# leonsick/s2d

Measured on AMD Instinct MI355X. Metric: clip-frames/sec fwd+loss, R50 M2F-Video T=8 720p Q=100, higher is better.
Workload: dtype f32 (f16x3 MFMA for dense contractions); 1 GPU; KDVideoMaskFormer fwd+loss (student+teacher fwd, GT+KD VideoSetCriterion), c4: 2 clips/GPU x T=8 x 720x1280, Q=100, P=160000, N=10 sparse GT instances/clip, encoder dropout 0.3; clips_per_gpu=2, frames_per_clip=8, parallelism=dp1 (clips sharded, no collective), streams=2

## Files before the change

### include/s2d_hip.h

```cpp
#ifndef S2D_HIP_H
#define S2D_HIP_H
#include <stdint.h>

#ifndef HIP_INCLUDE_HIP_HIP_RUNTIME_API_H
typedef struct ihipStream_t *hipStream_t;
#endif

#ifdef __cplusplus
extern "C" {
#endif

#define S2D_OK 0
#define S2D_ERR_ARG (-1)
#define S2D_ERR_LAUNCH (-2)

int s2d_abi_version(void);

int s2d_set_dense_mode(int mode);


int s2d_gemm_nt_f32(const float *A, const float *B, float *C, int M, int N, int K, long lda, long ldb, long ldc,
                    int batch, long strideA, long strideB, long strideC, const float *scale, const float *bias,
                    const float *res, long ldr, long strideR, int res_rows, int res_cols, int relu, const void *B_split,
                    hipStream_t stream);
// ... 259 lines not shown

int s2d_relu_gate_add_f32(const float *a, const float *g, const float *y, long n, float *out, hipStream_t stream);


int s2d_optim_grad_norm_f32(const void *const *ptrs, const long *numel, const int *chunk_tensor, const long *chunk_off,
                            int nchunks, int chunk, float inv_scale, float max_norm, double *partial, float *normbuf,
                            hipStream_t stream);

int s2d_optim_adamw_ema_f32(const void *const *ptrs, const long *numel, const double *hyper, const int *chunk_tensor,
                            const long *chunk_off, int nchunks, int chunk, double lr_factor, double beta1, double beta2,
                            double eps, double bias_correction1, double bias_correction2_sqrt, float inv_scale, double ema_m,
                            const float *normbuf, hipStream_t stream);

int s2d_point_loss_backward_f32(const float *mask_logits, const uint8_t *tgt, const int *tgt_count, const int *nonempty,
                                const int *idx_q, const int *idx_t, const int *n_match, const float *coords_over,
                                const float *coords_rand, uint64_t seed, int NL, int B, int Q, int ldq, int T, int hm, int wm,
                                int H, int W, int Nmax, int num_points, float oversample_ratio, float importance_ratio,
                                int drop_empty, float world_size, void *workspace, float w_mask, float w_dice, float *grad_rows,
                                unsigned int *bit_scratch, hipStream_t stream);

int s2d_point_loss_rng_points(uint64_t seed, int hm, int wm, int row0, int nrows, int n_over, float *uv, int *bounds, int *scratch_list,
                              hipStream_t stream);

int s2d_class_loss_backward_f32(const float *class_logits, const int *idx_q, const int *n_match, int B, int Q, int maxm,
                                float eos_coef, float w_ce, float *d_class_logits, hipStream_t stream);

int s2d_class_loss_backward_c_f32(const float *class_logits, int C1, const int *idx_q, const int *n_match, int B, int Q, int maxm,
                                  float eos_coef, float w_ce, float *d_class_logits, hipStream_t stream);


int s2d_tracks_to_masks_u8(const float *tracks, int T, int Np, int H, int W, uint8_t *masks, hipStream_t stream);

int s2d_point_id_counts(const uint8_t *point_masks, const int64_t *idmap, int T, int H, int W, int Hi, int Wi, int max_id,
                        int *counts, int *total, hipStream_t stream);

int s2d_track_point_id_counts(const float *tracks, int T, int P, int H, int W, const int64_t *idmap, int Hi, int Wi, int max_id,
                              int *counts, int *total, hipStream_t stream);

int s2d_idmap_select_masks_u8(const int64_t *idmap, int T, int H, int W, const int *frames, const int *objs, int K, uint8_t *out,
                              hipStream_t stream);

int s2d_idmap_presence_u8(const int64_t *idmap, int T, int Hi, int Wi, int max_id, uint8_t *presence, hipStream_t stream);

long s2d_color_ids_workspace_words(int T);
int s2d_color_masks_to_ids(const uint8_t *rgb, int T, int H, int W, unsigned int *workspace, int *n_ids, int64_t *ids,
                           int *overflow, hipStream_t stream);
// ... 64 lines not shown
```

### s2d_amd/csrc/loss.hip

```cpp
#include "common.h"
#include "class_select.h"

namespace {

__device__ __forceinline__ uint64_t mix64(uint64_t z)
{
    z += 0x9E3779B97F4A7C15ull;
    z = (z ^ (z >> 30)) * 0xBF58476D1CE4E5B9ull;
    z = (z ^ (z >> 27)) * 0x94D049BB133111EBull;
    return z ^ (z >> 31);
}
__device__ __forceinline__ uint32_t hash32(uint32_t x)
{
    x ^= x >> 16; x *= 0x7feb352du; x ^= x >> 15; x *= 0x846ca68bu; x ^= x >> 16;
    return x;
}
__device__ __forceinline__ uint32_t rand_key(uint64_t seed, uint64_t stream)
{
    return (uint32_t)mix64(seed ^ mix64(stream * 0xD1342543DE82EF95ull));
}
__device__ __forceinline__ uint32_t rand_u_bits(uint32_t key, uint32_t i) { return hash32(key + i); }
__device__ __forceinline__ uint32_t rand_v_bits(uint32_t a)
{
    uint32_t b = a * 0x9E3779B1u;
// ... 178 lines not shown
    const int *nonempty;
    const int *idx_q, *idx_t;
    const int *n_match;
    const float *coords_over;
    const float *coords_rand;
    uint64_t seed;
    int NL, B, Q, ldq, T, hm, wm, H, W, Nmax, maxm, n_over, n_unc, n_rand, drop;
    float world_size;
    int *active, *rank;
    int *list;
    int *lcount;
    float *mq;
    unsigned int *hist;
    unsigned int *prefix;
    int *krem;
    unsigned int *tie;
    float *part;
    int chunks;
    float *xbuf;
    unsigned int *tpack;
    int bits_global;
    int xcap;
    int *pbound;
};

__device__ __forceinline__ uint64_t key_row(const LossParams &p, long rowid)
{
    if (p.NL == 0) return (uint64_t)rowid;
    const long per = (long)p.maxm * p.T;
    const long lb = rowid / per;
    return (uint64_t)(lb * ((long)p.Q * p.T) + (rowid - lb * per));
}

constexpr int PB_STRIDE = 9;
struct VRange {
    float v0, dv;
};

__global__ void row_prep_kernel(LossParams p)
{
    const int layer = blockIdx.x;
    const int rows_l = p.B * p.maxm * p.T;
    __shared__ int base;
    if (threadIdx.x == 0) base = 0;
    __syncthreads();
    for (int r0 = 0; r0 < rows_l; r0 += blockDim.x) {
        const int r = r0 + threadIdx.x;
        int act = 0;
        if (r < rows_l) {
            const int t = r % p.T, s = (r / p.T) % p.maxm, b = r / (p.T * p.maxm);
            const int prob = layer * p.B + b;
            if (s < p.n_match[prob]) {
                const int n = p.idx_t[(long)prob * p.maxm + s];
                act = p.drop ? p.nonempty[((long)b * p.Nmax + n) * p.T + t] : 1;
            }
        }
        __shared__ int wsum[4];
        const unsigned long long m = __ballot(act);
        const int lane = threadIdx.x & 63, wv = threadIdx.x >> 6;
        const int inw = __popcll(m & ((1ull << lane) - 1ull));
        if (lane == 0) wsum[wv] = __popcll(m);
        __syncthreads();
        int off = base;
        for (int w = 0; w < wv; ++w) off += wsum[w];
        if (r < rows_l) {
            const long rowid = (long)layer * rows_l + r;
            p.active[rowid] = act;
// ... 271 lines not shown
{
    extern __shared__ __attribute__((aligned(16))) float smem[];
    __shared__ int hq_idx[LTHREADS / 64][128];
    __shared__ float hq_y[LTHREADS / 64][128];
    constexpr int nb = LEVEL == 0 ? 2048 : 1024;
    const PartGeom g = part_geom(p.hm, p.wm);
    unsigned int *h = reinterpret_cast<unsigned int *>(smem);
    float *sm = smem + 2048;
    PartIter it(p, g.nparts, LEVEL == 0 ? 0 : p.xcap);
    long rowid; int part, li;
    while (it.next(p, rowid, part, li)) {
        __syncthreads();
        for (int i = threadIdx.x; i < nb; i += LTHREADS) h[i] = 0u;
        const int r0 = part * g.rows_per_part;
        const int nr = min(g.rows_per_part + 1, p.hm - r0);
        const float *cr = coord_rows(p, rowid, true);
        const bool padded = cr == nullptr;
        const int wp = p.wm + 2 * PADC;
        if (padded) stage_part_padded(p.mq + rowid * p.hm * p.wm, p.wm, r0, nr, sm);
        else stage_part(p.mq + rowid * p.hm * p.wm, p.wm, r0, nr, sm);
        __syncthreads();
        const unsigned int pre = LEVEL > 0 ? p.prefix[rowid] : 0u;
        const uint32_t key0 = rand_key(p.seed, key_row(p, rowid) * 2);
        const int ylo = part == 0 ? -1 : r0, yhi = r0 + g.rows_per_part;
        auto tally = [&](int i, float xv) {
            const unsigned int key = __float_as_uint(fabsf(xv));
            if (LEVEL == 0 && li < p.xcap && !(S2D_LOSS_DBG & 4)) p.xbuf[(long)li * (p.n_over + p.n_rand) + i] = xv;
            if ((S2D_LOSS_DBG & 1) && LEVEL == 0) { if (key == 0x12345u) h[0] = 1u; return; }
            if (LEVEL == 0) atomicAdd(&h[key >> 20], 1u);
            else if (LEVEL == 1) { if ((key >> 20) == (pre >> 20)) atomicAdd(&h[(key >> 10) & 1023u], 1u); }
            else { if ((key >> 10) == (pre >> 10)) atomicAdd(&h[key & 1023u], 1u); }
        };
        if (!cr) {
            const int *pb = p.pbound + rowid * PB_STRIDE;
            const int lo = pb[part], hi = pb[part + 1];
            const VRange vr = part_vrange(part, g.nparts, g.rows_per_part, p.hm);
            const int y0max = min(yhi, p.hm) - 1;
#pragma unroll 2
            for (int i = lo + (int)threadIdx.x; i < hi; i += LTHREADS) {
                const uint32_t ra_ = rand_u_bits(key0, (uint32_t)i);
                const float u = (float)(ra_ >> 8) * (1.0f / 16777216.0f);
                const float v = fmaf((float)(rand_v_bits(ra_) >> 8) * (1.0f / 16777216.0f), vr.dv, vr.v0);
                const float y = ((2.f * v - 1.f + 1.f) * p.hm - 1.f) * 0.5f;
                const float x = ((2.f * u - 1.f + 1.f) * p.wm - 1.f) * 0.5f;
                const int y0 = min(max((int)floorf(y), ylo), y0max);
                if (S2D_LOSS_DBG & 2) tally(i, x * y + (float)y0); else
                tally(i, sample_part_padded(sm, wp, r0, x, y, (int)floorf(x), y0));
            }
        } else {
            const int lane = threadIdx.x & 63, wv = threadIdx.x >> 6;
            int *qi = hq_idx[wv];
            float *qy = hq_y[wv];
// ... 34 lines not shown
            const uint32_t key1 = rand_key(p.seed, key_row(p, rowid) * 2 + 1);
            for (int i = threadIdx.x; i < p.n_rand; i += LTHREADS) {
                float u, v;
                if (cr2) { u = cr2[2 * i]; v = cr2[2 * i + 1]; }
                else {
                    const uint32_t ra_ = rand_u_bits(key1, (uint32_t)i);
                    u = (float)(ra_ >> 8) * (1.0f / 16777216.0f);
                    v = (float)(rand_v_bits(ra_) >> 8) * (1.0f / 16777216.0f);
                }
                const float y = ((2.f * v - 1.f + 1.f) * p.hm - 1.f) * 0.5f;
                const float x = ((2.f * u - 1.f + 1.f) * p.wm - 1.f) * 0.5f;
                const int y0 = (int)floorf(y);
                if (y0 >= ylo && y0 < yhi)
                    p.xbuf[(long)li * (p.n_over + p.n_rand) + p.n_over + i] =
                        padded ? sample_part_padded(sm, wp, r0, x, y, (int)floorf(x), y0) : sample_part(sm, p.hm, p.wm, r0, nr, x, y, (int)floorf(x), y0);
            }
        }
        __syncthreads();
        for (int i = threadIdx.x; i < nb; i += LTHREADS)
            if (h[i]) atomicAdd(&p.hist[rowid * 2048 + i], h[i]);
    }
}

template <int LEVEL>
__global__ __launch_bounds__(256) void hist_stream_kernel(LossParams p)
{
    __shared__ unsigned int h[1024];
    constexpr int SCH = 8;
    const int nrows = min(p.lcount[p.NL], p.xcap);
    for (int w = blockIdx.x; w < nrows * SCH; w += gridDim.x) {
        const int li = w / SCH, chunk = w % SCH;
        const long rowid = p.list[li];
        __syncthreads();
        for (int i = threadIdx.x; i < 1024; i += 256) h[i] = 0u;
        __syncthreads();
        const unsigned int pre = p.prefix[rowid];
        const float *xb = p.xbuf + (long)li * (p.n_over + p.n_rand);
        const int per = ((p.n_over + SCH - 1) / SCH + 3) & ~3;
        const int i0 = chunk * per, i1 = min(p.n_over, i0 + per);
        for (int i = i0 + threadIdx.x * 4; i < i1; i += 256 * 4) {
            const f32x4 v = *reinterpret_cast<const f32x4 *>(xb + i);
#pragma unroll
            for (int j = 0; j < 4; ++j) {
                if (i + j >= i1) break;
                const unsigned int key = __float_as_uint(fabsf(v[j]));
                if (LEVEL == 1) { if ((key >> 20) == (pre >> 20)) atomicAdd(&h[(key >> 10) & 1023u], 1u); }
                else { if ((key >> 10) == (pre >> 10)) atomicAdd(&h[key & 1023u], 1u); }
            }
        }
        __syncthreads();
        for (int i = threadIdx.x; i < 1024; i += 256)
            if (h[i]) atomicAdd(&p.hist[rowid * 2048 + i], h[i]);
    }
}

template <bool COH = false>
__device__ __forceinline__ float sample_bits(const unsigned int *bits, int H, int W, float u, float v)
{
    const float gx = 2.f * u - 1.f, gy = 2.f * v - 1.f;
    const float x = ((gx + 1.f) * W - 1.f) * 0.5f, y = ((gy + 1.f) * H - 1.f) * 0.5f;
    const int x0 = (int)floorf(x), y0 = (int)floorf(y), x1 = x0 + 1, y1 = y0 + 1;
    const float fx = x - x0, fy = y - y0;
    const float wxa = (x0 >= 0 && x0 < W) ? 1.f - fx : 0.f, wxb = (x1 >= 0 && x1 < W) ? fx : 0.f;
    const float wya = (y0 >= 0 && y0 < H) ? 1.f - fy : 0.f, wyb = (y1 >= 0 && y1 < H) ? fy : 0.f;
    const int xa = min(max(x0, 0), W - 1), xb = min(max(x1, 0), W - 1);
    const int ya = min(max(y0, 0), H - 1) * W, yb = min(max(y1, 0), H - 1) * W;
    auto bit = [&](int idx) {
        const unsigned int w = COH ? __hip_atomic_load(bits + (idx >> 5), __ATOMIC_RELAXED, __HIP_MEMORY_SCOPE_AGENT) : bits[idx >> 5];
        return (float)((w >> (idx & 31)) & 1u);
    };
    float acc = bit(ya + xa) * (wxa * wya);
    acc += bit(ya + xb) * (wxb * wya);
    acc += bit(yb + xa) * (wxa * wyb);
    acc += bit(yb + xb) * (wxb * wyb);
    return acc;
}

template <int LEVEL>
__global__ __launch_bounds__(256) void select_kernel(LossParams p)
{
    __shared__ unsigned int csum[256];
    if ((int)blockIdx.x >= p.lcount[p.NL]) return;
    const long rowid = p.list[blockIdx.x];
    const int nb = LEVEL == 0 ? 2048 : 1024, per = nb / 256;
    const int k = LEVEL == 0 ? p.n_unc : p.krem[rowid];
    unsigned int *h = p.hist + rowid * 2048;
    unsigned int loc[8], s = 0;
    for (int j = 0; j < per; ++j) { loc[j] = h[threadIdx.x * per + j]; s += loc[j]; }
    csum[threadIdx.x] = s;
    __syncthreads();
    if (threadIdx.x == 0) {
        unsigned int run = 0;
        for (int i = 0; i < 256; ++i) { const unsigned int c = csum[i]; csum[i] = run; run += c; }
    }
    __syncthreads();
    unsigned int before = csum[threadIdx.x];
    if (k == 0 && LEVEL == 0 && threadIdx.x == 0) { p.prefix[rowid] = 0u; p.krem[rowid] = 0; }
    for (int j = 0; j < per; ++j) {
        if (before < (unsigned)k && before + loc[j] >= (unsigned)k) {
            const unsigned int bin = threadIdx.x * per + j;
            const unsigned int pre = LEVEL == 0 ? 0u : p.prefix[rowid];
            p.prefix[rowid] = LEVEL == 0 ? (bin << 20) : LEVEL == 1 ? (pre | (bin << 10)) : (pre | bin);
            p.krem[rowid] = k - (int)before;
        }
        before += loc[j];
    }
    __syncthreads();
    for (int j = 0; j < per; ++j) h[threadIdx.x * per + j] = 0u;
}

__device__ __forceinline__ void acc_point(float x, float t, float &bce, float &sgt, float &sg, float &ts)
{
    const float e = __expf(-fabsf(x));
    const float inv = __builtin_amdgcn_rcpf(1.f + e);
    const float s = x >= 0.f ? inv : e * inv;
    bce += fmaxf(x, 0.f) - x * t + __logf(1.f + e);
    sgt += s * t; sg += s; ts += t;
}

__global__ __launch_bounds__(LTHREADS) void accumulate_kernel(LossParams p)
{
    extern __shared__ __attribute__((aligned(16))) float smem[];
    __shared__ float red[LTHREADS / 64][4];
    const PartGeom g = part_geom(p.hm, p.wm);
    float *sm = smem;
    const int rows_l = p.B * p.maxm * p.T;
    PartIter it(p, g.nparts, p.xcap);
    long rowid; int part, li;
    while (it.next(p, rowid, part, li)) {
        __syncthreads();
        const int r0 = part * g.rows_per_part;
// ... 87 lines not shown
        out |= ((w4 & 0xFFu) ? 1u : 0u) << (4 * k);
        out |= ((w4 & 0xFF00u) ? 1u : 0u) << (4 * k + 1);
        out |= ((w4 & 0xFF0000u) ? 1u : 0u) << (4 * k + 2);
        out |= ((w4 & 0xFF000000u) ? 1u : 0u) << (4 * k + 3);
    }
    p.tpack[(long)plane * wpp + wd] = out;
}

struct LossBwdArgs {
    float *gplane;
    float w_mask, w_dice;
    unsigned int *bit_scratch;
};
template <bool BWD, bool GBITS = BWD>
__global__ __launch_bounds__(LTHREADS) void accumulate_stream_kernel(LossParams p, LossBwdArgs ba)
{
    extern __shared__ __attribute__((aligned(16))) unsigned int tbits[];
    __shared__ float red[LTHREADS / 64][4];
    constexpr int TIECAP = 512;
    __shared__ unsigned int tie_n, tie_base, wtie[LTHREADS / 64];
    __shared__ int tie_idx[TIECAP], tie_sorted[TIECAP];
    __shared__ int cq_idx[LTHREADS / 64][128];
    __shared__ float cq_val[LTHREADS / 64][128];
    const int rows_l = p.B * p.maxm * p.T;
    const int nrows = min(p.lcount[p.NL], p.xcap);
    const long HW = (long)p.H * p.W;
    __shared__ float s_v0[PB_STRIDE], s_dv[PB_STRIDE];
    __shared__ int s_pb[PB_STRIDE];
    const PartGeom sg_ = part_geom(p.hm, p.wm);
    if ((int)threadIdx.x < sg_.nparts) { const VRange vr = part_vrange(threadIdx.x, sg_.nparts, sg_.rows_per_part, p.hm); s_v0[threadIdx.x] = vr.v0; s_dv[threadIdx.x] = vr.dv; }
    static_assert(GBITS || !BWD, "the backward keeps its gradient tile in the dynamic LDS");
    const unsigned int *tb = tbits;
    int *gh = reinterpret_cast<int *>(tbits);
    const float n_pts = (float)(p.n_unc + p.n_rand);
    const bool injected = p.coords_over != nullptr || p.coords_rand != nullptr;
    const float FX_CAP = injected ? fmaxf(n_pts, 1.f) : fminf(fmaxf(n_pts, 1.f), fmaxf(1024.f, 256.f * n_pts / (float)(p.hm * p.wm)));
    __shared__ unsigned int tie_before;
    for (int li = blockIdx.x; li < nrows; li += gridDim.x) {
        const long rowid = p.list[li];
        const int layer = (int)(rowid / rows_l);
        const int r = (int)(rowid % rows_l);
        const int t = r % p.T, s = (r / p.T) % p.maxm, b = r / (p.T * p.maxm);
        const int prob = layer * p.B + b;
        const int n = p.idx_t[(long)prob * p.maxm + s];
        const unsigned int *pk = p.tpack + (((long)b * p.Nmax + n) * p.T + t) * (HW / 32);
        __syncthreads();
        if (threadIdx.x < PB_STRIDE) s_pb[threadIdx.x] = p.pbound[rowid * PB_STRIDE + threadIdx.x];
        if constexpr (GBITS) tb = pk;
        else {
#pragma unroll 4
            for (long w4 = threadIdx.x; w4 < HW / 128; w4 += LTHREADS) reinterpret_cast<uint4 *>(tbits)[w4] = reinterpret_cast<const uint4 *>(pk)[w4];
            for (long wd = (HW / 128) * 4 + threadIdx.x; wd < HW / 32; wd += LTHREADS) tbits[wd] = pk[wd];
        }
        if (threadIdx.x == 0) { tie_n = 0u; tie_base = 0u; }
        __syncthreads();
        const unsigned int thr = p.prefix[rowid];
        const unsigned int take = (unsigned int)p.krem[rowid];
        const float *xb = p.xbuf + (long)li * (p.n_over + p.n_rand);
        float bce = 0.f, sgt = 0.f, sg = 0.f, ts = 0.f;
        float g_bce = 0.f, g_dice = 0.f, dA = 0.f, dD = 1.f, fx_scale = 0.f, fx_inv = 0.f;
        float *gp = nullptr;
        if constexpr (BWD) {
            double num = 0.;
            for (int bb = 0; bb < p.B; ++bb) num += (double)min(p.tgt_count[bb], p.Nmax);
            num = fmax(num / (double)p.world_size, 1.0);
            float a = 0.f, bsum = 0.f, c = 0.f;
            for (int ch = 0; ch < p.chunks; ++ch) {
                const float *qd = p.part + (rowid * p.chunks + ch) * 4;
                a += qd[1]; bsum += qd[2]; c += qd[3];
            }
            dA = 2.f * a + 1.f; dD = bsum + c + 1.f;
            g_bce = ba.w_mask / ((float)num * (float)(p.n_unc + p.n_rand));
            g_dice = ba.w_dice / (float)num;
            gp = ba.gplane + rowid * (long)p.hm * p.wm;
            const float gmax = fabsf(g_bce) + fabsf(g_dice) * (2.f * dD + fabsf(dA)) / (4.f * dD * dD);
            fx_scale = gmax > 0.f ? exp2f(floorf(log2f(2147483648.f / (FX_CAP * gmax)))) : 0.f;
            fx_inv = fx_scale > 0.f ? 1.f / fx_scale : 0.f;
        }
        int ylo = 0, yhi = p.hm;
        int own_lo = -1, own_hi = p.hm;
// ... 74 lines not shown
                }
                point(xv, sample_bits(tb, p.H, p.W, u, v), u, v);
            };
            const int lane = threadIdx.x & 63, wv = threadIdx.x >> 6;
            int *qi = cq_idx[wv];
            float *qx = cq_val[wv];
            int qn = 0;
            auto push = [&](bool sel, int i, float xv) {
                const unsigned long long m = __ballot(sel);
                if (sel) {
                    const int pos = qn + (int)__popcll(m & ((1ull << lane) - 1ull));
                    qi[pos] = i; qx[pos] = xv;
                }
                qn += (int)__popcll(m);
                if (qn >= 64) {
                    heavy(qi[lane], qx[lane]);
                    const int rest = qn - 64;
                    int ti = 0; float tx = 0.f;
                    if (lane < rest) { ti = qi[64 + lane]; tx = qx[64 + lane]; }
                    if (lane < rest) { qi[lane] = ti; qx[lane] = tx; }
                    qn = rest;
                }
            };
            auto test = [&](int i, float xv, bool live) {
                const bool inr = live && i >= lo && i < hi;
                bool owned = inr;
                if (BWD && !walk_range && inr) {
                    float v;
                    if (cr) v = cr[2 * i + 1];
                    else if (over) { float u; over_point_rng(key0, i, s_pb, s_v0, s_dv, sg_.nparts, u, v); }
                    else v = (float)(rand_v_bits(rand_u_bits(key0, (uint32_t)i)) >> 8) * (1.0f / 16777216.0f);
                    const int y0 = y0_of(v);
                    owned = y0 >= own_lo && y0 < own_hi;
                }
                bool sel = owned;
                if (over) {
                    const unsigned int key = __float_as_uint(fabsf(xv));
                    sel = owned && key < thr;
                    if (inr && key == thr) {
                        const unsigned int slot = atomicAdd(&tie_n, 1u);
                        if (slot < TIECAP) tie_idx[slot] = i;
                    }
                }
                push(sel, i, xv);
            };
            const int cnt4 = ((reinterpret_cast<uintptr_t>(xs) & 15) == 0) ? cnt >> 2 : 0;
            const int b4 = min(lo >> 2, cnt4), e4 = min((hi + 3) >> 2, cnt4);
            const int it4 = (e4 - b4 + LTHREADS - 1) / LTHREADS;
            auto load4 = [&](int k) {
                const int i4 = b4 + k * LTHREADS + threadIdx.x;
                f32x4 x4 = {0.f, 0.f, 0.f, 0.f};
                if (i4 < e4) x4 = *reinterpret_cast<const f32x4 *>(xs + 4 * i4);
                return x4;
            };
            constexpr int DEPTH = 8;
            f32x4 ring[DEPTH];
#pragma unroll
            for (int d = 0; d < DEPTH; ++d) ring[d] = load4(d);
            for (int k0 = 0; k0 < it4; k0 += DEPTH) {
#pragma unroll
                for (int d = 0; d < DEPTH; ++d) {
                    const int k = k0 + d;
                    if (k >= it4) break;
                    const int i4 = b4 + k * LTHREADS + threadIdx.x;
                    const bool live = i4 < e4;
                    const f32x4 x4 = ring[d];
                    ring[d] = load4(k + DEPTH);
#pragma unroll
                    for (int j = 0; j < 4; ++j) test(4 * i4 + j, x4[j], live);
                }
            }
            const int tail0 = 4 * cnt4, itt = (cnt - tail0 + LTHREADS - 1) / LTHREADS;
            for (int k = 0; k < itt; ++k) {
                const int i = tail0 + k * LTHREADS + threadIdx.x;
                const bool live = i < cnt;
                test(i, live ? xs[i] : 0.f, live);
            }
            if (lane < qn) heavy(qi[lane], qx[lane]);
        }
        __syncthreads();
        const unsigned int nties = tie_n;
        const bool ranged_ties = BWD && ranged;
        const unsigned int before = ranged_ties ? tie_before : 0u;
        __syncthreads();
        if (ranged_ties && threadIdx.x == 0) tie_before = before + nties;
        if (nties > 0u && take > before) {
            const float *cr = coord_rows(p, rowid, true);
            const uint32_t key0 = rand_key(p.seed, key_row(p, rowid) * 2);
            auto tie_point = [&](int i) {
                float u, v;
                if (cr) { u = cr[2 * i]; v = cr[2 * i + 1]; }
                else over_point_rng(key0, i, s_pb, s_v0, s_dv, sg_.nparts, u, v);
                if (BWD && !ranged_ties) { const int y0 = y0_of(v); if (y0 < own_lo || y0 >= own_hi) return; }
                point(xb[i], sample_bits(tb, p.H, p.W, u, v), u, v);
            };
            if (nties <= (unsigned int)TIECAP) {
                for (unsigned int j = threadIdx.x; j < nties; j += LTHREADS) {
                    const int mine = tie_idx[j];
                    unsigned int rank = 0u;
// ... 28 lines not shown
            __syncthreads();
            const int nxt = part + 1 < nparts_b ? max((part + 1) * sg_.rows_per_part - 1, 0) : p.hm;
            for (int i = threadIdx.x; i < (min(nxt, yhi) - ylo) * p.wm; i += LTHREADS) gp[ylo * p.wm + i] = (float)gh[i] * fx_inv;
        }
        }
        if constexpr (!BWD) {
            bce = wave_sum(bce); sgt = wave_sum(sgt); sg = wave_sum(sg); ts = wave_sum(ts);
            const int lane = threadIdx.x & 63, wv = threadIdx.x >> 6;
            if (lane == 0) { red[wv][0] = bce; red[wv][1] = sgt; red[wv][2] = sg; red[wv][3] = ts; }
            __syncthreads();
            if (threadIdx.x < 4) {
                const int j = threadIdx.x;
                float tot = 0.f;
#pragma unroll
                for (int w = 0; w < LTHREADS / 64; ++w) tot += red[w][j];
                p.part[(rowid * p.chunks + 0) * 4 + j] = tot;
#pragma unroll 1
                for (int c = 1; c < p.chunks; ++c) p.part[(rowid * p.chunks + c) * 4 + j] = 0.f;
            }
        }
    }
}

__global__ void loss_finalize_kernel(LossParams p, float *__restrict__ losses)
{
    const int layer = blockIdx.x;
    if (threadIdx.x != 0) return;
    const int rows_l = p.B * p.maxm * p.T;
    double num = 0.;
    for (int b = 0; b < p.B; ++b) num += (double)min(p.tgt_count[b], p.Nmax);
    num = fmax(num / (double)p.world_size, 1.0);
    const double P = (double)(p.n_unc + p.n_rand);
    double lm = 0., ld = 0.;
    for (int r = 0; r < rows_l; ++r) {
        const long rowid = (long)layer * rows_l + r;
        if (!p.active[rowid]) continue;
        double bce = 0., sgt = 0., sg = 0., ts = 0.;
        for (int c = 0; c < p.chunks; ++c) {
            const float *q = p.part + (rowid * p.chunks + c) * 4;
            bce += q[0]; sgt += q[1]; sg += q[2]; ts += q[3];
        }
        lm += bce / P;
        ld += 1.0 - (2.0 * sgt + 1.0) / (sg + ts + 1.0);
    }
    losses[layer * 2 + 0] = (float)(lm / num);
    losses[layer * 2 + 1] = (float)(ld / num);
// ... 203 lines not shown

int s2d_target_nonempty(const uint8_t *tgt, const int *count, int B, int Nmax, int T, int H, int W, int *nonempty,
                        hipStream_t stream)
{
    if (B * Nmax * T == 0) return S2D_OK;
    if (((long)H * W) % 16) return S2D_ERR_ARG;
    if (s2d_zero_async(nonempty, sizeof(int) * (size_t)B * Nmax * T, stream) != S2D_OK) return S2D_ERR_LAUNCH;
    hipLaunchKernelGGL(nonempty_kernel, dim3(B * Nmax * T, NE_CHUNKS), dim3(256), 0, stream, tgt, count, Nmax, T, (long)H * W, nonempty);
    S2D_CHECK_LAUNCH();
    return S2D_OK;
}

static const int LOSS_CHUNKS = 8;

static const long XBUF_MAX_ROWS = 4096;

static void point_counts(int num_points, float oversample_ratio, float importance_ratio, int &n_over, int &n_unc, int &n_rand)
{
    n_over = (int)(num_points * oversample_ratio);
    n_unc = (int)(importance_ratio * num_points);
    n_rand = num_points - n_unc;
}

static inline bool plane_in_lds(long HW) { return HW / 8 <= 140 * 1024; }
constexpr int ACC_BLOCKS = 512;

long s2d_point_loss_workspace_bytes(int NL, int B, int Q, int Nmax, int T, int hm, int wm, int num_points,
                                    float oversample_ratio, float importance_ratio, int H, int W)
{
    const long maxm = Q < Nmax ? Q : Nmax;
    const long rows = (long)NL * B * maxm * T;
    int n_over, n_unc, n_rand;
    point_counts(num_points, oversample_ratio, importance_ratio, n_over, n_unc, n_rand);
    const long xrows = rows < XBUF_MAX_ROWS ? rows : XBUF_MAX_ROWS;
    const long HW = (long)H * W;
    return rows * (3 * 4 + (long)hm * wm * 4 + 2048 * 4 + 4 + 4 + 4 + LOSS_CHUNKS * 16 + PB_STRIDE * 4) + 4L * (NL + 1) + 1024 +
           xrows * (long)(n_over + n_rand + 8) * 4 + 256 + (long)B * Nmax * T * (HW / 32 + 1) * 4;
}

static int loss_setup(LossParams &p, long &rows, const float *mask_logits, const uint8_t *tgt, const int *tgt_count, const int *nonempty,
                      const int *idx_q, const int *idx_t, const int *n_match, const float *coords_over, const float *coords_rand,
                      uint64_t seed, int NL, int B, int Q, int ldq, int T, int hm, int wm, int H, int W, int Nmax, int num_points,
                      float oversample_ratio, float importance_ratio, int drop_empty, float world_size, void *workspace)
{
    if (Q > 128 || Nmax > 128 || ldq > 128 || ldq < Q || (ldq & 3)) return S2D_ERR_ARG;
    p.ml = mask_logits; p.tgt = tgt; p.tgt_count = tgt_count; p.nonempty = nonempty;
    p.idx_q = idx_q; p.idx_t = idx_t; p.n_match = n_match; p.coords_over = coords_over; p.coords_rand = coords_rand;
    p.seed = seed; p.NL = NL; p.B = B; p.Q = Q; p.ldq = ldq; p.T = T; p.hm = hm; p.wm = wm; p.H = H; p.W = W; p.Nmax = Nmax;
    p.maxm = Q < Nmax ? Q : Nmax;
    point_counts(num_points, oversample_ratio, importance_ratio, p.n_over, p.n_unc, p.n_rand);
    p.drop = drop_empty; p.world_size = world_size; p.chunks = LOSS_CHUNKS;
    rows = (long)NL * B * p.maxm * T;
    if (rows == 0) return S2D_OK;
    char *w = (char *)workspace;
    p.active = (int *)w; w += rows * 4;
    p.rank = (int *)w; w += rows * 4;
    p.prefix = (unsigned int *)w; w += rows * 4;
    p.krem = (int *)w; w += rows * 4;
    p.tie = (unsigned int *)w; w += rows * 4;
    p.list = (int *)w; w += rows * 4;
    p.lcount = (int *)w; w += 4L * (NL + 1);
    w = (char *)(((uintptr_t)w + 255) & ~(uintptr_t)255);
    p.hist = (unsigned int *)w; w += rows * 2048 * 4;
    p.part = (float *)w; w += rows * LOSS_CHUNKS * 16;
    p.pbound = (int *)w; w += rows * PB_STRIDE * 4;
    p.mq = (float *)w; w += rows * (long)hm * wm * 4;
    w = (char *)(((uintptr_t)w + 255) & ~(uintptr_t)255);
    p.xbuf = (float *)w;
    const bool can_stream = (p.n_over % 4 == 0) && (p.n_rand % 4 == 0) && ((long)H * W % 32 == 0);
    p.xcap = can_stream ? (int)(rows < XBUF_MAX_ROWS ? rows : XBUF_MAX_ROWS) : 0;
    {
        char *e = (char *)p.xbuf + (long)(rows < XBUF_MAX_ROWS ? rows : XBUF_MAX_ROWS) * (p.n_over + p.n_rand + 8) * 4;
        p.tpack = (unsigned int *)(((uintptr_t)e + 255) & ~(uintptr_t)255);
    }
    p.bits_global = can_stream && !plane_in_lds((long)H * W);
    const PartGeom pg = part_geom(hm, wm);
    if ((wm & 3) || pg.rows_per_part < 1 || pg.nparts > LOSS_CHUNKS) return S2D_ERR_ARG;
    p.chunks = pg.nparts;
    return S2D_OK;
}

static int loss_attrs()
{
    static S2dDevOnce attr_set;
    if (!attr_set.done()) {
        const int cap = PART_BYTES + 8192 + 4096;
        if (hipFuncSetAttribute(reinterpret_cast<const void *>(hist_kernel<0>), hipFuncAttributeMaxDynamicSharedMemorySize, cap) != hipSuccess ||
            hipFuncSetAttribute(reinterpret_cast<const void *>(hist_kernel<1>), hipFuncAttributeMaxDynamicSharedMemorySize, cap) != hipSuccess ||
            hipFuncSetAttribute(reinterpret_cast<const void *>(hist_kernel<2>), hipFuncAttributeMaxDynamicSharedMemorySize, cap) != hipSuccess ||
            hipFuncSetAttribute(reinterpret_cast<const void *>(accumulate_kernel), hipFuncAttributeMaxDynamicSharedMemorySize, cap) != hipSuccess ||
            hipFuncSetAttribute(reinterpret_cast<const void *>(accumulate_stream_kernel<false>), hipFuncAttributeMaxDynamicSharedMemorySize, 140 * 1024) != hipSuccess ||
            hipFuncSetAttribute(reinterpret_cast<const void *>(accumulate_stream_kernel<false, true>), hipFuncAttributeMaxDynamicSharedMemorySize, 140 * 1024) != hipSuccess ||
            hipFuncSetAttribute(reinterpret_cast<const void *>(accumulate_stream_kernel<true>), hipFuncAttributeMaxDynamicSharedMemorySize, 140 * 1024) != hipSuccess)
            return S2D_ERR_LAUNCH;
        attr_set.mark();
    }
    return S2D_OK;
}

int s2d_point_loss_f32(const float *mask_logits, const uint8_t *tgt, const int *tgt_count, const int *nonempty,
                       const int *idx_q, const int *idx_t, const int *n_match, const float *coords_over,
                       const float *coords_rand, uint64_t seed, int NL, int B, int Q, int ldq, int T, int hm, int wm, int H,
                       int W, int Nmax, int num_points, float oversample_ratio, float importance_ratio, int drop_empty,
                       float world_size, void *workspace, float *losses, hipStream_t stream)
{
    LossParams p;
    long rows = 0;
    if (int e = loss_setup(p, rows, mask_logits, tgt, tgt_count, nonempty, idx_q, idx_t, n_match, coords_over, coords_rand, seed, NL, B, Q, ldq,
                           T, hm, wm, H, W, Nmax, num_points, oversample_ratio, importance_ratio, drop_empty, world_size, workspace))
        return e;
    if (rows == 0) return S2D_OK;
    if (s2d_zero_async(p.hist, (size_t)rows * 2048 * 4, stream) != S2D_OK) return S2D_ERR_LAUNCH;
    if (s2d_zero_async(p.tie, (size_t)rows * 4, stream) != S2D_OK) return S2D_ERR_LAUNCH;
    hipLaunchKernelGGL(row_prep_kernel, dim3(NL), dim3(256), 0, stream, p);
    hipLaunchKernelGGL(row_list_kernel, dim3(NL), dim3(256), 0, stream, p);
    hipLaunchKernelGGL(gather_rows_kernel, dim3(cdiv((long)hm * wm, 64), T, NL * B), dim3(256), 0, stream, p);
    const PartGeom pg = part_geom(hm, wm);
    static_assert(PB_STRIDE == LOSS_CHUNKS + 1, "one bound per part + the end");
    if (!coords_over) hipLaunchKernelGGL(row_strata_kernel, dim3(cdiv(rows, 4)), dim3(256), 0, stream, p, pg.nparts, pg.rows_per_part);
    const size_t lds_map = sizeof(float) * (size_t)(pg.rows_per_part + 3) * (wm + 2 * PADC);
    const size_t lds_hist = lds_map + sizeof(float) * 2048;
    if (int e = loss_attrs()) return e;
    const dim3 g(512);
    hipLaunchKernelGGL(hist_kernel<0>, g, dim3(LTHREADS), lds_hist, stream, p);
    hipLaunchKernelGGL(select_kernel<0>, dim3((unsigned)rows), dim3(256), 0, stream, p);
    if (p.xcap > 0) hipLaunchKernelGGL(hist_stream_kernel<1>, dim3(2048), dim3(256), 0, stream, p);
    if (rows > p.xcap) hipLaunchKernelGGL(hist_kernel<1>, g, dim3(LTHREADS), lds_hist, stream, p);
    hipLaunchKernelGGL(select_kernel<1>, dim3((unsigned)rows), dim3(256), 0, stream, p);
    if (p.xcap > 0) hipLaunchKernelGGL(hist_stream_kernel<2>, dim3(2048), dim3(256), 0, stream, p);
    if (rows > p.xcap) hipLaunchKernelGGL(hist_kernel<2>, g, dim3(LTHREADS), lds_hist, stream, p);
    hipLaunchKernelGGL(select_kernel<2>, dim3((unsigned)rows), dim3(256), 0, stream, p);
    if (p.xcap > 0)
        hipLaunchKernelGGL(pack_planes_kernel, dim3(cdiv((long)H * W / 32, 256), B * Nmax * T), dim3(256), 0, stream, p);
    if (p.xcap > 0 && !p.bits_global)
        hipLaunchKernelGGL(accumulate_stream_kernel<false>, dim3(ACC_BLOCKS), dim3(LTHREADS), (size_t)((long)H * W / 8), stream, p, LossBwdArgs{nullptr, 0.f, 0.f, nullptr});
    else if (p.xcap > 0)
        hipLaunchKernelGGL((accumulate_stream_kernel<false, true>), dim3(ACC_BLOCKS), dim3(LTHREADS), 16, stream, p, LossBwdArgs{nullptr, 0.f, 0.f, nullptr});
    if (rows > p.xcap) hipLaunchKernelGGL(accumulate_kernel, g, dim3(LTHREADS), lds_map, stream, p);
    hipLaunchKernelGGL(loss_finalize_kernel, dim3(NL), dim3(64), 0, stream, p, losses);
    S2D_CHECK_LAUNCH();
    return S2D_OK;
}

int s2d_point_loss_backward_f32(const float *mask_logits, const uint8_t *tgt, const int *tgt_count, const int *nonempty,
                                const int *idx_q, const int *idx_t, const int *n_match, const float *coords_over,
                                const float *coords_rand, uint64_t seed, int NL, int B, int Q, int ldq, int T, int hm, int wm, int H,
                                int W, int Nmax, int num_points, float oversample_ratio, float importance_ratio, int drop_empty,
                                float world_size, void *workspace, float w_mask, float w_dice, float *grad_rows,
                                unsigned int *bit_scratch, hipStream_t stream)
{
    LossParams p;
    long rows = 0;
    if (int e = loss_setup(p, rows, mask_logits, tgt, tgt_count, nonempty, idx_q, idx_t, n_match, coords_over, coords_rand, seed, NL, B, Q, ldq,
                           T, hm, wm, H, W, Nmax, num_points, oversample_ratio, importance_ratio, drop_empty, world_size, workspace))
        return e;
    if (rows == 0) return S2D_OK;
    if (p.xcap <= 0) return S2D_ERR_ARG;
    if (int e = loss_attrs()) return e;
    if (s2d_zero_async(grad_rows, sizeof(float) * (size_t)rows * hm * wm, stream) != S2D_OK) return S2D_ERR_LAUNCH;
    const PartGeom pg = part_geom(hm, wm);
// ... 2 lines not shown
    hipLaunchKernelGGL(accumulate_stream_kernel<true>, dim3(ACC_BLOCKS), dim3(LTHREADS), lds, stream, p,
                       LossBwdArgs{grad_rows, w_mask, w_dice, bit_scratch});
    S2D_CHECK_LAUNCH();
    return S2D_OK;
}

int s2d_point_loss_rng_points(uint64_t seed, int hm, int wm, int row0, int nrows, int n_over, float *uv, int *bounds, int *scratch_list,
                              hipStream_t stream)
{
    const PartGeom pg = part_geom(hm, wm);
    if ((wm & 3) || pg.rows_per_part < 1 || pg.nparts > LOSS_CHUNKS || nrows <= 0 || row0 != 0) return S2D_ERR_ARG;
    LossParams p = {};
    p.seed = seed; p.hm = hm; p.wm = wm; p.n_over = n_over; p.NL = 0;
    p.list = scratch_list;
    p.lcount = scratch_list + nrows;
    p.pbound = bounds;
    hipLaunchKernelGGL(rng_points_prep_kernel, dim3(cdiv(nrows + 1, 256)), dim3(256), 0, stream, scratch_list, nrows);
    hipLaunchKernelGGL(row_strata_kernel, dim3(cdiv(nrows, 4)), dim3(256), 0, stream, p, pg.nparts, pg.rows_per_part);
    hipLaunchKernelGGL(rng_points_kernel, dim3(cdiv(n_over, 256), nrows), dim3(256), 0, stream, p, pg.nparts, pg.rows_per_part, uv);
    S2D_CHECK_LAUNCH();
    return S2D_OK;
}

int s2d_class_loss_backward_f32(const float *class_logits, const int *idx_q, const int *n_match, int B, int Q, int maxm, float eos_coef,
                                float w_ce, float *d_class_logits, hipStream_t stream)
{
    if (Q > 128) return S2D_ERR_ARG;
    hipLaunchKernelGGL(class_loss_backward_kernel, dim3(1), dim3(128), 0, stream, class_logits, idx_q, n_match, B, Q, maxm, eos_coef, w_ce,
                       d_class_logits);
    S2D_CHECK_LAUNCH();
    return S2D_OK;
}

int s2d_class_loss_f32(const float *class_logits, const int *idx_q, const int *n_match, int B, int Q, int maxm,
                       float eos_coef, float *loss_ce, hipStream_t stream)
{
    if (Q > 128) return S2D_ERR_ARG;
    hipLaunchKernelGGL(class_loss_kernel, dim3(1), dim3(128), 0, stream, class_logits, idx_q, n_match, B, Q, maxm, eos_coef,
                       loss_ce);
    S2D_CHECK_LAUNCH();
    return S2D_OK;
}

int s2d_class_loss_c_f32(const float *class_logits, int C1, const int *idx_q, const int *n_match, int B, int Q, int maxm,
                         float eos_coef, float *loss_ce, hipStream_t stream)
{
// ... 20 lines not shown
```

Baseline: 176.4 clip-frames/s.

## Fuse point-loss top-k threshold refinement into accumulate kernel via fine histogram

For rows whose oversampled logits are buffered, the first histogram pass now uses a finer 2048-bin log-scaled key range. The accumulate kernel collects the candidates that fall in the threshold bin into per-wave LDS buffers and refines the exact k-th threshold in place. This replaces the two extra global hist/select levels and their kernel launches. Rows with too many candidates or edge bins fall back to an exact in-block radix select kernel. The cost is extra LDS in the accumulate kernel, possible re-scans when a buffer overflows, and more complex selection logic.

New measurement: 176.2 clip-frames/s. Within noise of the previous version (-0.1%).

```diff
diff --git a/include/s2d_hip.h b/include/s2d_hip.h
--- a/include/s2d_hip.h
+++ b/include/s2d_hip.h
@@ -305,6 +305,9 @@
 int s2d_point_loss_rng_points(uint64_t seed, int hm, int wm, int row0, int nrows, int n_over, float *uv, int *bounds, int *scratch_list,
                               hipStream_t stream);
 
+int s2d_point_loss_select_stats(const void *workspace, int NL, int B, int Q, int Nmax, int T, int hm, int wm, int num_points,
+                                float oversample_ratio, float importance_ratio, int H, int W, int *out, hipStream_t stream);
+
 int s2d_class_loss_backward_f32(const float *class_logits, const int *idx_q, const int *n_match, int B, int Q, int maxm,
                                 float eos_coef, float w_ce, float *d_class_logits, hipStream_t stream);
 
diff --git a/s2d_amd/csrc/loss.hip b/s2d_amd/csrc/loss.hip
--- a/s2d_amd/csrc/loss.hip
+++ b/s2d_amd/csrc/loss.hip
@@ -224,7 +224,22 @@
     int bits_global;
     int xcap;
     int *pbound;
+    int *fstat;
+    int *flist;
 };
+
+constexpr int FINE_SHIFT = 15;
+constexpr int FINE_LO = (127 - 4) << 8;
+constexpr int FINE_BINS = 2048;
+constexpr int CAND_CAP = 2560;
+constexpr int CAND_WCAP = 384;
+constexpr int CAND_BYTES = (512 / 64) * CAND_WCAP * 8;
+constexpr unsigned int CAND_FLAG = 0x80000000u;
+enum { FS_MARKED = 0, FS_MAXCAND = 1, FS_OVERFLOW = 2 };
+__device__ __forceinline__ unsigned int fine_bin(unsigned int key)
+{
+    return (unsigned int)min(max((int)(key >> FINE_SHIFT) - FINE_LO, 0), FINE_BINS - 1);
+}
 
 __device__ __forceinline__ uint64_t key_row(const LossParams &p, long rowid)
 {
@@ -245,6 +260,7 @@
     const int rows_l = p.B * p.maxm * p.T;
     __shared__ int base;
     if (threadIdx.x == 0) base = 0;
+    if (layer == 0 && threadIdx.x < 8) p.fstat[threadIdx.x] = 0;
     __syncthreads();
     for (int r0 = 0; r0 < rows_l; r0 += blockDim.x) {
         const int r = r0 + threadIdx.x;
@@ -562,12 +578,13 @@
         __syncthreads();
         const unsigned int pre = LEVEL > 0 ? p.prefix[rowid] : 0u;
         const uint32_t key0 = rand_key(p.seed, key_row(p, rowid) * 2);
+        const bool fine = LEVEL == 0 && li < p.xcap;
         const int ylo = part == 0 ? -1 : r0, yhi = r0 + g.rows_per_part;
         auto tally = [&](int i, float xv) {
             const unsigned int key = __float_as_uint(fabsf(xv));
             if (LEVEL == 0 && li < p.xcap && !(S2D_LOSS_DBG & 4)) p.xbuf[(long)li * (p.n_over + p.n_rand) + i] = xv;
             if ((S2D_LOSS_DBG & 1) && LEVEL == 0) { if (key == 0x12345u) h[0] = 1u; return; }
-            if (LEVEL == 0) atomicAdd(&h[key >> 20], 1u);
+            if (LEVEL == 0) atomicAdd(&h[fine ? fine_bin(key) : key >> 20], 1u);
             else if (LEVEL == 1) { if ((key >> 20) == (pre >> 20)) atomicAdd(&h[(key >> 10) & 1023u], 1u); }
             else { if ((key >> 10) == (pre >> 10)) atomicAdd(&h[key & 1023u], 1u); }
         };
@@ -648,35 +665,70 @@
     }
 }
 
-template <int LEVEL>
-__global__ __launch_bounds__(256) void hist_stream_kernel(LossParams p)
-{
-    __shared__ unsigned int h[1024];
-    constexpr int SCH = 8;
-    const int nrows = min(p.lcount[p.NL], p.xcap);
-    for (int w = blockIdx.x; w < nrows * SCH; w += gridDim.x) {
-        const int li = w / SCH, chunk = w % SCH;
+__device__ __forceinline__ void find_kth_bin(const unsigned int *h, int nb, unsigned int k, unsigned int *res)
+{
+    if (threadIdx.x < 64) {
+        const int lane = threadIdx.x, per = nb >> 6;
+        unsigned int s = 0u;
+        for (int j = 0; j < per; ++j) s += h[lane * per + j];
+        unsigned int inc = s;
+#pragma unroll
+        for (int o = 1; o < 64; o <<= 1) {
+            const unsigned int t = __shfl_up(inc, o, 64);
+            if (lane >= o) inc += t;
+        }
+        unsigned int before = inc - s;
+        if (before < k && inc >= k) {
+            for (int j = 0; j < per; ++j) {
+                const unsigned int c = h[lane * per + j];
+                if (before + c >= k) { res[0] = lane * per + j; res[1] = before; res[2] = c; break; }
+                before += c;
+            }
+        }
+    }
+    __syncthreads();
+}
+
+template <int NT>
+__device__ void exact_select(const float *__restrict__ xs, int n, int k, unsigned int *h, unsigned int *res, unsigned int &key_out, unsigned int &take_out)
+{
+    unsigned int pre = 0u, kr = (unsigned int)k;
+#pragma unroll 1
+    for (int level = 0; level < 3; ++level) {
+        const int nb = level == 0 ? 2048 : 1024;
+        __syncthreads();
+        for (int i = threadIdx.x; i < nb; i += NT) h[i] = 0u;
+        if (threadIdx.x < 3) res[threadIdx.x] = 0u;
+        __syncthreads();
+        for (int i = threadIdx.x * 4; i < n; i += NT * 4) {
+            const f32x4 v = *reinterpret_cast<const f32x4 *>(xs + i);
+#pragma unroll
+            for (int j = 0; j < 4; ++j) {
+                const unsigned int key = __float_as_uint(fabsf(v[j]));
+                if (level == 0) atomicAdd(&h[key >> 20], 1u);
+                else if (level == 1) { if ((key >> 20) == (pre >> 20)) atomicAdd(&h[(key >> 10) & 1023u], 1u); }
+                else { if ((key >> 10) == (pre >> 10)) atomicAdd(&h[key & 1023u], 1u); }
+            }
+        }
+        __syncthreads();
+        find_kth_bin(h, nb, kr, res);
+        pre |= res[0] << (level == 0 ? 20 : level == 1 ? 10 : 0);
+        kr -= res[1];
+    }
+    key_out = pre; take_out = kr;
+}
+
+__global__ __launch_bounds__(LTHREADS) void select_fallback_kernel(LossParams p)
+{
+    __shared__ unsigned int h[2048];
+    __shared__ unsigned int res[4];
+    const int nmark = p.fstat[FS_MARKED];
+    for (int m = blockIdx.x; m < nmark; m += gridDim.x) {
+        const int li = p.flist[m];
         const long rowid = p.list[li];
-        __syncthreads();
-        for (int i = threadIdx.x; i < 1024; i += 256) h[i] = 0u;
-        __syncthreads();
-        const unsigned int pre = p.prefix[rowid];
-        const float *xb = p.xbuf + (long)li * (p.n_over + p.n_rand);
-        const int per = ((p.n_over + SCH - 1) / SCH + 3) & ~3;
-        const int i0 = chunk * per, i1 = min(p.n_over, i0 + per);
-        for (int i = i0 + threadIdx.x * 4; i < i1; i += 256 * 4) {
-            const f32x4 v = *reinterpret_cast<const f32x4 *>(xb + i);
-#pragma unroll
-            for (int j = 0; j < 4; ++j) {
-                if (i + j >= i1) break;
-                const unsigned int key = __float_as_uint(fabsf(v[j]));
-                if (LEVEL == 1) { if ((key >> 20) == (pre >> 20)) atomicAdd(&h[(key >> 10) & 1023u], 1u); }
-                else { if ((key >> 10) == (pre >> 10)) atomicAdd(&h[key & 1023u], 1u); }
-            }
-        }
-        __syncthreads();
-        for (int i = threadIdx.x; i < 1024; i += 256)
-            if (h[i]) atomicAdd(&p.hist[rowid * 2048 + i], h[i]);
+        unsigned int key, take;
+        exact_select<LTHREADS>(p.xbuf + (long)li * (p.n_over + p.n_rand), p.n_over, p.n_unc, h, res, key, take);
+        if (threadIdx.x == 0) { p.prefix[rowid] = key; p.krem[rowid] = (int)take; }
     }
 }
 
@@ -707,6 +759,8 @@
 {
     __shared__ unsigned int csum[256];
     if ((int)blockIdx.x >= p.lcount[p.NL]) return;
+    const bool stored = (int)blockIdx.x < p.xcap;
+    if (LEVEL > 0 && stored) return;
     const long rowid = p.list[blockIdx.x];
     const int nb = LEVEL == 0 ? 2048 : 1024, per = nb / 256;
     const int k = LEVEL == 0 ? p.n_unc : p.krem[rowid];
@@ -726,13 +780,23 @@
         if (before < (unsigned)k && before + loc[j] >= (unsigned)k) {
             const unsigned int bin = threadIdx.x * per + j;
             const unsigned int pre = LEVEL == 0 ? 0u : p.prefix[rowid];
-            p.prefix[rowid] = LEVEL == 0 ? (bin << 20) : LEVEL == 1 ? (pre | (bin << 10)) : (pre | bin);
-            p.krem[rowid] = k - (int)before;
+            if (LEVEL == 0 && stored) {
+                const bool mark = loc[j] > (unsigned)CAND_CAP || bin == 0u || bin == (unsigned)(FINE_BINS - 1);
+                p.tie[rowid] = loc[j];
+                atomicMax(&p.fstat[FS_MAXCAND], (int)loc[j]);
+                if (mark) p.flist[atomicAdd(&p.fstat[FS_MARKED], 1)] = (int)blockIdx.x;
+                p.prefix[rowid] = mark ? 0u : (CAND_FLAG | bin);
+                p.krem[rowid] = mark ? 0 : k - (int)before;
+            } else {
+                p.prefix[rowid] = LEVEL == 0 ? (bin << 20) : LEVEL == 1 ? (pre | (bin << 10)) : (pre | bin);
+                p.krem[rowid] = k - (int)before;
+            }
         }
         before += loc[j];
     }
     __syncthreads();
-    for (int j = 0; j < per; ++j) h[threadIdx.x * per + j] = 0u;
+    if (!stored)
+        for (int j = 0; j < per; ++j) h[threadIdx.x * per + j] = 0u;
 }
 
 __device__ __forceinline__ void acc_point(float x, float t, float &bce, float &sgt, float &sg, float &ts)
@@ -866,9 +930,11 @@
     __shared__ int tie_idx[TIECAP], tie_sorted[TIECAP];
     __shared__ int cq_idx[LTHREADS / 64][128];
     __shared__ float cq_val[LTHREADS / 64][128];
+    __shared__ unsigned int wcn[LTHREADS / 64], sres[4];
     const int rows_l = p.B * p.maxm * p.T;
     const int nrows = min(p.lcount[p.NL], p.xcap);
     const long HW = (long)p.H * p.W;
+    unsigned int *cand = tbits + (GBITS ? 0 : (HW / 32 + 3) / 4 * 4);
     __shared__ float s_v0[PB_STRIDE], s_dv[PB_STRIDE];
     __shared__ int s_pb[PB_STRIDE];
     const PartGeom sg_ = part_geom(p.hm, p.wm);
@@ -898,8 +964,11 @@
         }
         if (threadIdx.x == 0) { tie_n = 0u; tie_base = 0u; }
         __syncthreads();
-        const unsigned int thr = p.prefix[rowid];
-        const unsigned int take = (unsigned int)p.krem[rowid];
+        unsigned int thr = p.prefix[rowid];
+        unsigned int take = (unsigned int)p.krem[rowid];
+        int mode = 0;
+        unsigned int b0 = 0u;
+        if constexpr (!BWD) if (thr & CAND_FLAG) { mode = 1; b0 = thr & (unsigned)(FINE_BINS - 1); }
         const float *xb = p.xbuf + (long)li * (p.n_over + p.n_rand);
         float bce = 0.f, sgt = 0.f, sg = 0.f, ts = 0.f;
         float g_bce = 0.f, g_dice = 0.f, dA = 0.f, dD = 1.f, fx_scale = 0.f, fx_inv = 0.f;
@@ -1020,6 +1089,9 @@
                     qn = rest;
                 }
             };
+            int *ci = reinterpret_cast<int *>(cand) + wv * CAND_WCAP;
+            float *cv = reinterpret_cast<float *>(cand) + (LTHREADS / 64 + wv) * CAND_WCAP;
+            int cn = 0;
             auto test = [&](int i, float xv, bool live) {
                 const bool inr = live && i >= lo && i < hi;
                 bool owned = inr;
@@ -1031,16 +1103,35 @@
                     const int y0 = y0_of(v);
                     owned = y0 >= own_lo && y0 < own_hi;
                 }
-                bool sel = owned;
+                bool sel = owned, isc = false;
                 if (over) {
                     const unsigned int key = __float_as_uint(fabsf(xv));
-                    sel = owned && key < thr;
-                    if (inr && key == thr) {
+                    bool below = key < thr, tied = key == thr;
+                    if constexpr (!BWD) {
+                        if (mode != 0) {
+                            const unsigned int bin = fine_bin(key);
+                            isc = inr && bin == b0;
+                            below = mode == 1 ? bin < b0 : isc && below;
+                            tied = mode == 2 && tied;
+                        }
+                    }
+                    sel = owned && below;
+                    if (inr && tied) {
                         const unsigned int slot = atomicAdd(&tie_n, 1u);
                         if (slot < TIECAP) tie_idx[slot] = i;
                     }
                 }
                 push(sel, i, xv);
+                if constexpr (!BWD) {
+                    if (mode == 1) {
+                        const unsigned long long m = __ballot(isc);
+                        if (isc) {
+                            const int pos = cn + (int)__popcll(m & ((1ull << lane) - 1ull));
+                            if (pos < CAND_WCAP) { ci[pos] = i; cv[pos] = xv; }
+                        }
+                        cn += (int)__popcll(m);
+                    }
+                }
             };
             const int cnt4 = ((reinterpret_cast<uintptr_t>(xs) & 15) == 0) ? cnt >> 2 : 0;
             const int b4 = min(lo >> 2, cnt4), e4 = min((hi + 3) >> 2, cnt4);
@@ -1053,6 +1144,9 @@
             };
             constexpr int DEPTH = 8;
             f32x4 ring[DEPTH];
+#pragma unroll 1
+            for (;;) {
+            cn = 0;
 #pragma unroll
             for (int d = 0; d < DEPTH; ++d) ring[d] = load4(d);
             for (int k0 = 0; k0 < it4; k0 += DEPTH) {
@@ -1073,6 +1167,57 @@
                 const int i = tail0 + k * LTHREADS + threadIdx.x;
                 const bool live = i < cnt;
                 test(i, live ? xs[i] : 0.f, live);
+            }
+            if (BWD || !over || mode != 1) break;
+            if constexpr (!BWD) {
+                if (lane == 0) wcn[wv] = (unsigned int)cn;
+                __syncthreads();
+                bool fits = true;
+#pragma unroll
+                for (int w = 0; w < LTHREADS / 64; ++w) fits = fits && wcn[w] <= (unsigned)CAND_WCAP;
+                if (fits) {
+                    unsigned int *hh = reinterpret_cast<unsigned int *>(tie_sorted);
+                    unsigned int sub = 0u;
+                    constexpr int LO_BITS = FINE_SHIFT - 8;
+                    constexpr unsigned int LO_MASK = (1u << LO_BITS) - 1u;
+#pragma unroll 1
+                    for (int lvl = 0; lvl < 2; ++lvl) {
+                        if (threadIdx.x < 256) hh[threadIdx.x] = 0u;
+                        if (threadIdx.x < 3) sres[threadIdx.x] = 0u;
+                        __syncthreads();
+                        for (int j = lane; j < cn; j += 64) {
+                            const unsigned int key = __float_as_uint(fabsf(cv[j]));
+                            if (lvl == 0) atomicAdd(&hh[(key >> LO_BITS) & 255u], 1u);
+                            else if (((key >> LO_BITS) & 255u) == sub) atomicAdd(&hh[key & LO_MASK], 1u);
+                        }
+                        __syncthreads();
+                        find_kth_bin(hh, 256, take, sres);
+                        sub = lvl == 0 ? sres[0] : (sub << LO_BITS) | sres[0];
+                        take -= sres[1];
+                        __syncthreads();
+                    }
+                    thr = ((b0 + (unsigned)FINE_LO) << FINE_SHIFT) | sub;
+                } else {
+                    exact_select<LTHREADS>(xb, p.n_over, p.n_unc, cand, sres, thr, take);
+                    if (threadIdx.x == 0) atomicAdd(&p.fstat[FS_OVERFLOW], 1);
+                }
+                if (threadIdx.x == 0) { p.prefix[rowid] = thr; p.krem[rowid] = (int)take; }
+                if (!fits) { mode = 2; __syncthreads(); continue; }
+                mode = 0;
+                for (int j0 = 0; j0 < cn; j0 += 64) {
+                    const int j = j0 + lane;
+                    const bool livec = j < cn;
+                    const int i = livec ? ci[j] : 0;
+                    const float xv = livec ? cv[j] : 0.f;
+                    const unsigned int key = __float_as_uint(fabsf(xv));
+                    if (livec && key == thr) {
+                        const unsigned int slot = atomicAdd(&tie_n, 1u);
+                        if (slot < TIECAP) tie_idx[slot] = i;
+                    }
+                    push(livec && key < thr, i, xv);
+                }
+            }
+            break;
             }
             if (lane < qn) heavy(qi[lane], qx[lane]);
         }
@@ -1147,6 +1292,13 @@
     }
 }
 
+__global__ void select_stats_kernel(LossParams p, int *__restrict__ out)
+{
+    if (threadIdx.x != 0) return;
+    out[0] = min(p.lcount[p.NL], p.xcap);
+    out[1] = p.fstat[FS_MARKED]; out[2] = p.fstat[FS_MAXCAND]; out[3] = p.fstat[FS_OVERFLOW]; out[4] = CAND_CAP;
+}
+
 __global__ void loss_finalize_kernel(LossParams p, float *__restrict__ losses)
 {
     const int layer = blockIdx.x;
@@ -1396,7 +1548,9 @@
     n_rand = num_points - n_unc;
 }
 
-static inline bool plane_in_lds(long HW) { return HW / 8 <= 140 * 1024; }
+constexpr int ACC_DYN_LDS = 140 * 1024;
+static inline long plane_lds_bytes(long HW) { return (HW / 32 + 3) / 4 * 16; }
+static inline bool plane_in_lds(long HW) { return plane_lds_bytes(HW) + CAND_BYTES <= ACC_DYN_LDS; }
 constexpr int ACC_BLOCKS = 512;
 
 long s2d_point_loss_workspace_bytes(int NL, int B, int Q, int Nmax, int T, int hm, int wm, int num_points,
@@ -1409,7 +1563,8 @@
     const long xrows = rows < XBUF_MAX_ROWS ? rows : XBUF_MAX_ROWS;
     const long HW = (long)H * W;
     return rows * (3 * 4 + (long)hm * wm * 4 + 2048 * 4 + 4 + 4 + 4 + LOSS_CHUNKS * 16 + PB_STRIDE * 4) + 4L * (NL + 1) + 1024 +
-           xrows * (long)(n_over + n_rand + 8) * 4 + 256 + (long)B * Nmax * T * (HW / 32 + 1) * 4;
+           xrows * (long)(n_over + n_rand + 8) * 4 + 256 + (long)B * Nmax * T * (HW / 32 + 1) * 4 +
+           64 + 8 * 4 + xrows * 4;
 }
 
 static int loss_setup(LossParams &p, long &rows, const float *mask_logits, const uint8_t *tgt, const int *tgt_count, const int *nonempty,
@@ -1446,6 +1601,9 @@
     {
         char *e = (char *)p.xbuf + (long)(rows < XBUF_MAX_ROWS ? rows : XBUF_MAX_ROWS) * (p.n_over + p.n_rand + 8) * 4;
         p.tpack = (unsigned int *)(((uintptr_t)e + 255) & ~(uintptr_t)255);
+        e = (char *)(p.tpack + (long)B * Nmax * T * ((long)H * W / 32));
+        p.fstat = (int *)(((uintptr_t)e + 15) & ~(uintptr_t)15);
+        p.flist = p.fstat + 8;
     }
     p.bits_global = can_stream && !plane_in_lds((long)H * W);
     const PartGeom pg = part_geom(hm, wm);
@@ -1463,8 +1621,8 @@
             hipFuncSetAttribute(reinterpret_cast<const void *>(hist_kernel<1>), hipFuncAttributeMaxDynamicSharedMemorySize, cap) != hipSuccess ||
             hipFuncSetAttribute(reinterpret_cast<const void *>(hist_kernel<2>), hipFuncAttributeMaxDynamicSharedMemorySize, cap) != hipSuccess ||
             hipFuncSetAttribute(reinterpret_cast<const void *>(accumulate_kernel), hipFuncAttributeMaxDynamicSharedMemorySize, cap) != hipSuccess ||
-            hipFuncSetAttribute(reinterpret_cast<const void *>(accumulate_stream_kernel<false>), hipFuncAttributeMaxDynamicSharedMemorySize, 140 * 1024) != hipSuccess ||
-            hipFuncSetAttribute(reinterpret_cast<const void *>(accumulate_stream_kernel<false, true>), hipFuncAttributeMaxDynamicSharedMemorySize, 140 * 1024) != hipSuccess ||
+            hipFuncSetAttribute(reinterpret_cast<const void *>(accumulate_stream_kernel<false>), hipFuncAttributeMaxDynamicSharedMemorySize, ACC_DYN_LDS) != hipSuccess ||
+            hipFuncSetAttribute(reinterpret_cast<const void *>(accumulate_stream_kernel<false, true>), hipFuncAttributeMaxDynamicSharedMemorySize, ACC_DYN_LDS) != hipSuccess ||
             hipFuncSetAttribute(reinterpret_cast<const void *>(accumulate_stream_kernel<true>), hipFuncAttributeMaxDynamicSharedMemorySize, 140 * 1024) != hipSuccess)
             return S2D_ERR_LAUNCH;
         attr_set.mark();
@@ -1498,18 +1656,19 @@
     const dim3 g(512);
     hipLaunchKernelGGL(hist_kernel<0>, g, dim3(LTHREADS), lds_hist, stream, p);
     hipLaunchKernelGGL(select_kernel<0>, dim3((unsigned)rows), dim3(256), 0, stream, p);
-    if (p.xcap > 0) hipLaunchKernelGGL(hist_stream_kernel<1>, dim3(2048), dim3(256), 0, stream, p);
-    if (rows > p.xcap) hipLaunchKernelGGL(hist_kernel<1>, g, dim3(LTHREADS), lds_hist, stream, p);
-    hipLaunchKernelGGL(select_kernel<1>, dim3((unsigned)rows), dim3(256), 0, stream, p);
-    if (p.xcap > 0) hipLaunchKernelGGL(hist_stream_kernel<2>, dim3(2048), dim3(256), 0, stream, p);
-    if (rows > p.xcap) hipLaunchKernelGGL(hist_kernel<2>, g, dim3(LTHREADS), lds_hist, stream, p);
-    hipLaunchKernelGGL(select_kernel<2>, dim3((unsigned)rows), dim3(256), 0, stream, p);
+    if (p.xcap > 0) hipLaunchKernelGGL(select_fallback_kernel, dim3(256), dim3(LTHREADS), 0, stream, p);
+    if (rows > p.xcap) {
+        hipLaunchKernelGGL(hist_kernel<1>, g, dim3(LTHREADS), lds_hist, stream, p);
+        hipLaunchKernelGGL(select_kernel<1>, dim3((unsigned)rows), dim3(256), 0, stream, p);
+        hipLaunchKernelGGL(hist_kernel<2>, g, dim3(LTHREADS), lds_hist, stream, p);
+        hipLaunchKernelGGL(select_kernel<2>, dim3((unsigned)rows), dim3(256), 0, stream, p);
+    }
     if (p.xcap > 0)
         hipLaunchKernelGGL(pack_planes_kernel, dim3(cdiv((long)H * W / 32, 256), B * Nmax * T), dim3(256), 0, stream, p);
     if (p.xcap > 0 && !p.bits_global)
-        hipLaunchKernelGGL(accumulate_stream_kernel<false>, dim3(ACC_BLOCKS), dim3(LTHREADS), (size_t)((long)H * W / 8), stream, p, LossBwdArgs{nullptr, 0.f, 0.f, nullptr});
+        hipLaunchKernelGGL(accumulate_stream_kernel<false>, dim3(ACC_BLOCKS), dim3(LTHREADS), (size_t)(plane_lds_bytes((long)H * W) + CAND_BYTES), stream, p, LossBwdArgs{nullptr, 0.f, 0.f, nullptr});
     else if (p.xcap > 0)
-        hipLaunchKernelGGL((accumulate_stream_kernel<false, true>), dim3(ACC_BLOCKS), dim3(LTHREADS), 16, stream, p, LossBwdArgs{nullptr, 0.f, 0.f, nullptr});
+        hipLaunchKernelGGL((accumulate_stream_kernel<false, true>), dim3(ACC_BLOCKS), dim3(LTHREADS), CAND_BYTES, stream, p, LossBwdArgs{nullptr, 0.f, 0.f, nullptr});
     if (rows > p.xcap) hipLaunchKernelGGL(accumulate_kernel, g, dim3(LTHREADS), lds_map, stream, p);
     hipLaunchKernelGGL(loss_finalize_kernel, dim3(NL), dim3(64), 0, stream, p, losses);
     S2D_CHECK_LAUNCH();
@@ -1558,6 +1717,20 @@
     return S2D_OK;
 }
 
+int s2d_point_loss_select_stats(const void *workspace, int NL, int B, int Q, int Nmax, int T, int hm, int wm, int num_points,
+                                float oversample_ratio, float importance_ratio, int H, int W, int *out, hipStream_t stream)
+{
+    LossParams p;
+    long rows = 0;
+    if (int e = loss_setup(p, rows, nullptr, nullptr, nullptr, nullptr, nullptr, nullptr, nullptr, nullptr, nullptr, 0, NL, B, Q, 128, T, hm, wm, H, W,
+                           Nmax, num_points, oversample_ratio, importance_ratio, 0, 1.f, const_cast<void *>(workspace)))
+        return e;
+    if (rows == 0) return S2D_ERR_ARG;
+    hipLaunchKernelGGL(select_stats_kernel, dim3(1), dim3(64), 0, stream, p, out);
+    S2D_CHECK_LAUNCH();
+    return S2D_OK;
+}
+
 int s2d_class_loss_backward_f32(const float *class_logits, const int *idx_q, const int *n_match, int B, int Q, int maxm, float eos_coef,
                                 float w_ce, float *d_class_logits, hipStream_t stream)
 {
```
